# ZooMEISTER/vickers-hardness-Unet

Hardware: AMD Instinct MI355X
Metric: 512x512 images/sec (train fwd+bwd) (higher is better)
Workload: dtype bf16

## Files before the change

### include/vk_unet.h

```cpp
#ifndef VK_UNET_H
#define VK_UNET_H

#include <stddef.h>
#include <stdint.h>

#ifdef __cplusplus
extern "C" {
#endif

#define VK_ABI_VERSION 1
#define VK_STATS_REPLICAS 32

typedef enum { VK_F32 = 0, VK_BF16 = 1, VK_F16 = 2 } vk_dtype;

enum { VK_OK = 0, VK_ERR_ARG = -1, VK_ERR_STATE = -2, VK_ERR_UNSUPPORTED = -3 };

int vk_version(void);
const char* vk_last_error_string(void);
int vk_has_gfx950_code(void);
int vk_probe_mfma_rate(int iters, int waves_per_simd, float* sink, double* flops_out, void* stream);
int vk_set_reserved_cus(int n);
int vk_debug_hold_cus(int workgroups, int threads, int lds_bytes, int microseconds, const void* traffic, size_t traffic_bytes,
                      float* sink, void* stream);

// ... 27 lines not shown
int vk_conv_dgrad_pool2(const vk_conv_desc* d, const void* w, void* y_half, void* y1, int split_k1, int accumulate,
                        void* stream);

int vk_halo_pack(vk_dtype dtype, int rows, int red, const void* src, void* dst, void* stream);
int vk_conv_uses_halo_pack(const vk_conv_desc* d);
int vk_conv_fwd_packed(const vk_conv_desc* d, const void* w_halo, void* y, void* y1, int split_k1, int accumulate, double* stats,
                       void* stream);

#define VK_SPLITK_WORKSPACE_BYTES (32u << 20)
int vk_conv_fwd_splitk(const vk_conv_desc* d, const void* w_halo, void* y, void* workspace, size_t workspace_bytes, void* stream);

typedef struct {
  const void* z;
  const float* scale;
  const float* shift;
  double* sums;
  const void* mask;
  int accumulate;
} vk_bnr;

int vk_conv_dgrad_fused(const vk_conv_desc* d, const void* w, void* y, void* y1, int split_k1, int pool2, const vk_bnr* bnr,
                        void* stream);

int vk_conv1x1_fwd(const vk_conv_desc* d, const void* w, void* y, int accumulate, double* stats, void* stream);
int vk_conv1x1_wgrad(const vk_conv_desc* d, const void* dz, float* dw, void* workspace, size_t workspace_bytes, void* stream);

int vk_stem_fwd(vk_dtype dtype, int N, int H, int W, const void* x4, const void* wp, void* y, double* stats,
                void* stream);

#define VK_WGRAD_WORKSPACE_BYTES (64u << 20)
int vk_conv_wgrad(const vk_conv_desc* d, const void* dz, float* dw, void* workspace, size_t workspace_bytes, void* stream);
#define VK_WGRAD_BATCH_TABLE_BYTES (128u << 10)
int vk_conv_wgrad_batch_supports(const vk_conv_desc* d);
int vk_conv_wgrad_batch(const vk_conv_desc* descs, const void* const* dz, float* const* dw, int n, int workgroups, void* tables,
                        size_t tables_bytes, void* workspace, size_t workspace_bytes, void* stream);
int vk_stem_wgrad(vk_dtype dtype, int N, int H, int W, const void* x4, const void* dz, float* dw_krsc3, void* workspace,
                  size_t workspace_bytes, void* stream);
int vk_stem_wgrad_bn(vk_dtype dtype, int N, int H, int W, const void* x4, const void* g, const void* z, const float* coef_abc,
                     float* dw_krsc3, void* workspace, size_t workspace_bytes, void* stream);
int vk_stem_wgrad_c(vk_dtype dtype, int N, int H, int W, int cin, const void* x4, const void* dz, float* dw_krsc, void* workspace,
                    size_t workspace_bytes, void* stream);
int vk_stem_wgrad_bn_c(vk_dtype dtype, int N, int H, int W, int cin, const void* x4, const void* g, const void* z, const float* coef_abc,
                       float* dw_krsc, void* workspace, size_t workspace_bytes, void* stream);
int vk_conv_bwd_onepass(const vk_conv_desc* d_fwd, const void* g, const void* z, const float* coef_abc, const void* w_dgrad, void* y,
                        const vk_bnr* bnr, float* dw, void* workspace, size_t workspace_bytes, void* stream);
int vk_stem_dgrad(vk_dtype dtype, int N, int H, int W, const void* g, const void* z, const float* coef_abc, const float* w_krsc3,
                  float* dx, void* stream);
int vk_stem_dgrad_c(vk_dtype dtype, int N, int H, int W, int cin, const void* g, const void* z, const float* coef_abc, const float* w_krsc,
// ... 587 lines not shown
  int dims[4];
  int ndim;
  int64_t offset;
  int64_t numel;
} vk_tensor_info;

int vk_unet_create(const vk_unet_config* cfg, vk_unet** out);
int vk_unet_create_ex(const vk_unet_config* cfg, int classes, vk_unet** out);
int vk_unet_num_classes(const vk_unet* h);
#define VK_ENC_RESNET18 18
#define VK_ENC_RESNET34 34
#define VK_ENC_RESNET50 50
int vk_unet_create_enc(const vk_unet_config* cfg, int classes, int encoder, vk_unet** out);
int vk_unet_encoder(const vk_unet* h);
int vk_unet_create_in(const vk_unet_config* cfg, int classes, int encoder, int in_channels, vk_unet** out);
int vk_unet_in_channels(const vk_unet* h);
void vk_unet_destroy(vk_unet* h);
int vk_unet_set_side_stream(vk_unet* h, int enable);
int vk_unet_num_tensors(const vk_unet* h);
int vk_unet_tensor_info(const vk_unet* h, int index, vk_tensor_info* out);
int64_t vk_unet_param_numel(const vk_unet* h);
int64_t vk_unet_buffer_numel(const vk_unet* h);
int64_t vk_unet_workspace_bytes(const vk_unet* h);
int vk_unet_num_buckets(const vk_unet* h);
int vk_unet_bucket_range(const vk_unet* h, int bucket, int64_t* elem_begin, int64_t* elem_end);

int vk_unet_bind(vk_unet* h, float* params, float* grads, float* bn_buffers, int64_t* nbt, void* workspace,
                 size_t workspace_bytes);
int vk_unet_refresh_weights(vk_unet* h, void* stream);

int vk_unet_forward(vk_unet* h, const float* x, float* logits, int training, void* stream);
int vk_unet_loss(vk_unet* h, const float* logits, const float* target, float* loss_out, float grad_scale,
                 float w_bce, float w_dice, void* stream);
#define VK_LOSS_BINARY 0
#define VK_LOSS_MULTILABEL 1
#define VK_LOSS_MULTICLASS 2
int vk_unet_loss_ex(vk_unet* h, int mode, const void* logits, const void* target, float* loss_out, float grad_scale, float w_ce,
                    float w_dice, void* stream);
int vk_unet_loss_cfg(vk_unet* h, const vk_seg_loss_cfg* cfg, const void* logits, const void* target, float* loss_out,
                     float grad_scale, void* stream);
int vk_unet_loss_lovasz(vk_unet* h, const vk_seg_loss_cfg* seg_cfg, const vk_lovasz_cfg* lovasz_cfg, float w_lovasz, const void* logits,
                        const void* target, void* workspace, size_t workspace_bytes, float* loss_out, float grad_scale, void* stream);
int vk_unet_loss_kp(vk_unet* h, const vk_seg_loss_cfg* seg_cfg, const vk_kp_loss_cfg* kp_cfg, const void* logits, const void* target,
                    void* workspace, size_t workspace_bytes, float* loss_out, float grad_scale, void* stream);
int vk_unet_backward(vk_unet* h, const float* dlogits, int stage_begin, int stage_end, void* stream);
int vk_unet_set_trainable(vk_unet* h, const uint8_t* flags, int n);
// ... 20 lines not shown
```

### vickers-hardness-unet_amd/_lib.py

```python
from __future__ import annotations

import ctypes as C
import os
import subprocess
from pathlib import Path

PKG_DIR = Path(__file__).resolve().parent
LIB_PATH = Path(os.environ["VK_LIB"]) if os.environ.get("VK_LIB") else PKG_DIR / "libvkunet.so"
CSRC = PKG_DIR / "csrc"

VK_F32, VK_BF16, VK_F16 = 0, 1, 2
VK_LOSS_BINARY, VK_LOSS_MULTILABEL, VK_LOSS_MULTICLASS = 0, 1, 2
VK_ENC_RESNET18, VK_ENC_RESNET34, VK_ENC_RESNET50 = 18, 34, 50
VK_ADAMW_MAX_GROUPS = 8
VK_NORM_L2, VK_NORM_INF = 0, 1
VK_TILE_MAX_ORIGINS, VK_TILE_MAX_SIDE = 64, 4096
VK_BLEND_PROB, VK_BLEND_LOGIT = 0, 1
VK_PATCH_FORCE_GENERAL = 1


class VkError(RuntimeError):
    pass


# ... 264 lines not shown
vp, ci, cf, cd, sz, i64 = C.c_void_p, C.c_int, C.c_float, C.c_double, C.c_size_t, C.c_int64
P = C.POINTER

SIGNATURES = {
    "vk_version": (ci, []),
    "vk_last_error_string": (C.c_char_p, []),
    "vk_has_gfx950_code": (ci, []),
    "vk_probe_mfma_rate": (ci, [ci, ci, vp, P(C.c_double), vp]),
    "vk_set_reserved_cus": (ci, [ci]),
    "vk_debug_hold_cus": (ci, [ci, ci, ci, ci, vp, sz, vp, vp]),
    "vk_debug_set_stamp_buffer": (ci, [vp]),
    "vk_prof_enable": (ci, [ci]),
    "vk_prof_collect": (ci, [C.c_char_p, sz]),
    "vk_conv_fwd": (ci, [P(vk_conv_desc), vp, vp, vp, ci, ci, vp, vp]),
    "vk_conv_dgrad_pool2": (ci, [P(vk_conv_desc), vp, vp, vp, ci, ci, vp]),
    "vk_conv_dgrad_fused": (ci, [P(vk_conv_desc), vp, vp, vp, ci, ci, P(vk_bnr), vp]),
    "vk_head_bwd_fused": (ci, [ci, ci, ci, ci, P(vk_src), vp, vp, vp, vp, vp, P(vk_bnr), vp, sz, vp]),
    "vk_halo_pack": (ci, [ci, ci, ci, vp, vp, vp]),
    "vk_conv_uses_halo_pack": (ci, [P(vk_conv_desc)]),
    "vk_conv_fwd_packed": (ci, [P(vk_conv_desc), vp, vp, vp, ci, ci, vp, vp]),
    "vk_conv_fwd_splitk": (ci, [P(vk_conv_desc), vp, vp, vp, sz, vp]),
    "vk_stem_fwd": (ci, [ci, ci, ci, ci, vp, vp, vp, vp, vp]),
    "vk_conv_wgrad": (ci, [P(vk_conv_desc), vp, vp, vp, sz, vp]),
    "vk_conv1x1_fwd": (ci, [P(vk_conv_desc), vp, vp, ci, vp, vp]),
    "vk_conv1x1_wgrad": (ci, [P(vk_conv_desc), vp, vp, vp, sz, vp]),
    "vk_conv_wgrad_batch_supports": (ci, [P(vk_conv_desc)]),
    "vk_conv_wgrad_batch": (ci, [P(vk_conv_desc), P(vp), P(vp), ci, ci, vp, sz, vp, sz, vp]),
    "vk_stem_wgrad": (ci, [ci, ci, ci, ci, vp, vp, vp, vp, sz, vp]),
    "vk_stem_wgrad_bn": (ci, [ci, ci, ci, ci, vp, vp, vp, vp, vp, vp, sz, vp]),
    "vk_stem_wgrad_c": (ci, [ci, ci, ci, ci, ci, vp, vp, vp, vp, sz, vp]),
    "vk_stem_wgrad_bn_c": (ci, [ci, ci, ci, ci, ci, vp, vp, vp, vp, vp, vp, sz, vp]),
    "vk_conv_bwd_onepass": (ci, [P(vk_conv_desc), vp, vp, vp, vp, vp, P(vk_bnr), vp, vp, sz, vp]),
    "vk_stem_dgrad": (ci, [ci, ci, ci, ci, vp, vp, vp, vp, vp, vp]),
    "vk_stem_dgrad_c": (ci, [ci, ci, ci, ci, ci, vp, vp, vp, vp, vp, vp]),
    "vk_letterbox_preprocess": (ci, [P(vk_letterbox_desc), vp, vp, vp]),
    "vk_letterbox_postprocess_mask": (ci, [P(vk_letterbox_desc), vp, cf, vp, vp]),
    "vk_letterbox_postprocess_prob": (ci, [P(vk_letterbox_desc), vp, vp, vp]),
    "vk_letterbox_postprocess_labels": (ci, [P(vk_letterbox_desc), ci, vp, vp, vp]),
    "vk_letterbox_postprocess_mask_multi": (ci, [P(vk_letterbox_desc), ci, vp, cf, vp, vp]),
    "vk_letterbox_postprocess_prob_multi": (ci, [P(vk_letterbox_desc), ci, ci, vp, vp, vp]),
    "vk_tile_preprocess": (ci, [P(vk_tile_desc), vp, vp, vp]),
    "vk_tile_blend": (ci, [P(vk_tile_desc), ci, vp, cf, vp, vp, vp]),
    "vk_geom_workspace_bytes": (i64, [P(vk_geom_desc), ci]),
    "vk_geom_minarearect": (ci, [P(vk_geom_desc), ci, vp, vp, vp, vp, vp, sz, vp]),
    "vk_geom_quadrilateral": (ci, [P(vk_geom_desc), ci, ci, vp, vp, vp, vp, vp, sz, vp]),
    "vk_geom_slot_map": (ci, [P(vk_geom_desc), ci, vp, sz, vp, vp]),
    "vk_letterbox_u8": (ci, [P(vk_letterbox_desc), vp, vp, vp]),
    "vk_letterbox_mask_u8": (ci, [P(vk_letterbox_desc), vp, vp, vp]),
# ... 76 lines not shown
    "vk_adamw_step_amp": (ci, [sz, vp, vp, vp, vp, cf, cf, cf, cf, cf, vp, cf, vp, vp, vp, vp, ci, vp]),
    "vk_adamw_segment_blocks": (ci, [ci, P(i64), P(C.c_int32), ci]),
    "vk_adamw_step_amp_segments": (ci, [ci, vp, ci, vp, vp, vp, vp, vp, cf, cf, cf, cf, cf, vp, cf, vp, vp, vp, vp]),
    "vk_adamw_step_groups": (ci, [ci, vp, vp, ci, vp, vp, vp, vp, vp, ci, P(vk_adamw_group), vp, cf, vp, vp, vp, vp, vp]),
    "vk_grad_norm_segments": (ci, [ci, vp, ci, vp, vp, ci, cf, cf, vp, vp, vp]),
    "vk_avg_update": (ci, [ci, P(vk_avg_range), vk_avg_rule, vp, vp, vp, vp]),
    "vk_avg_swap": (ci, [ci, P(vk_avg_range), vp]),
    "vk_adamw_step_amp_avg": (ci, [sz, vp, vp, vp, vp, cf, cf, cf, cf, cf, vp, cf, vp, vp, vp, vp, ci, vp, vp, vk_avg_rule, vp, vp, vp, sz,
                                   vp]),
    "vk_unet_create": (ci, [P(vk_unet_config), P(vp)]),
    "vk_unet_create_ex": (ci, [P(vk_unet_config), ci, P(vp)]),
    "vk_unet_num_classes": (ci, [vp]),
    "vk_unet_create_enc": (ci, [P(vk_unet_config), ci, ci, P(vp)]),
    "vk_unet_encoder": (ci, [vp]),
    "vk_unet_create_in": (ci, [P(vk_unet_config), ci, ci, ci, P(vp)]),
    "vk_unet_in_channels": (ci, [vp]),
    "vk_unet_destroy": (None, [vp]),
    "vk_unet_set_side_stream": (ci, [vp, ci]),
    "vk_unet_num_tensors": (ci, [vp]),
    "vk_unet_tensor_info": (ci, [vp, ci, P(vk_tensor_info)]),
    "vk_unet_param_numel": (i64, [vp]),
    "vk_unet_buffer_numel": (i64, [vp]),
    "vk_unet_workspace_bytes": (i64, [vp]),
    "vk_unet_num_buckets": (ci, [vp]),
    "vk_unet_bucket_range": (ci, [vp, ci, P(i64), P(i64)]),
    "vk_unet_bind": (ci, [vp, vp, vp, vp, vp, vp, sz]),
    "vk_unet_refresh_weights": (ci, [vp, vp]),
    "vk_unet_forward": (ci, [vp, vp, vp, ci, vp]),
    "vk_unet_loss": (ci, [vp, vp, vp, vp, cf, cf, cf, vp]),
    "vk_unet_loss_ex": (ci, [vp, ci, vp, vp, vp, cf, cf, cf, vp]),
    "vk_unet_loss_cfg": (ci, [vp, P(vk_seg_loss_cfg), vp, vp, vp, cf, vp]),
    "vk_unet_loss_lovasz": (ci, [vp, P(vk_seg_loss_cfg), P(vk_lovasz_cfg), cf, vp, vp, vp, sz, vp, cf, vp]),
    "vk_unet_loss_kp": (ci, [vp, P(vk_seg_loss_cfg), P(vk_kp_loss_cfg), vp, vp, vp, sz, vp, cf, vp]),
    "vk_unet_backward": (ci, [vp, vp, ci, ci, vp]),
    "vk_unet_set_trainable": (ci, [vp, P(C.c_uint8), ci]),
    "vk_unet_set_bn_frozen": (ci, [vp, P(C.c_uint8), ci]),
    "vk_unet_set_input_grad": (ci, [vp, vp]),
    "vk_unet_zero_grad": (ci, [vp, vp]),
    "vk_unet_debug_tensor": (ci, [vp, C.c_char_p, P(vp), P(ci * 4)]),
    "vk_comm_unique_id": (ci, [vp]),
    "vk_comm_init": (ci, [ci, ci, vp, P(vp)]),
    "vk_comm_world": (ci, [vp]),
    "vk_allreduce_bucket": (ci, [vp, vp, sz, vp]),
    "vk_comm_broadcast": (ci, [vp, vp, sz, ci, vp]),
    "vk_comm_destroy": (ci, [vp]),
}
# ... 73 lines not shown
```

### vickers-hardness-unet_amd/csrc/elementwise.hip

```cpp
#include <math.h>

#include "vk_common.h"

namespace vk {

constexpr int kWideC = 2048;
static inline int channel_grid(int blocks, int cv) {
  int g = cv, r = 256;
  while (r) { const int t = g % r; g = r; r = t; }
  const int m = cv / g;
  return (blocks + m - 1) / m * m;
}

template <typename T>
__global__ void k_input_transform(int N, int cin, int H, int W, const float* __restrict__ x, T* __restrict__ x4) {
  const size_t HW = (size_t)H * W;
  const float* xn = x + (size_t)blockIdx.y * cin * HW;
  T* on = x4 + (size_t)blockIdx.y * HW * 4;
  for (size_t hw = blockIdx.x * (size_t)blockDim.x + threadIdx.x; hw < HW; hw += (size_t)gridDim.x * blockDim.x) {
    const float r = xn[hw], g = cin > 1 ? xn[HW + hw] : 0.f, b = cin > 2 ? xn[2 * HW + hw] : 0.f, a = cin > 3 ? xn[3 * HW + hw] : 0.f;
    if constexpr (sizeof(T) == 4) {
      *reinterpret_cast<f32x4_t*>(on + hw * 4) = f32x4_t{r, g, b, a};
    } else {
      float f[8] = {r, g, b, a, 0.f, 0.f, 0.f, 0.f};
// ... 438 lines not shown
                                                              const float* __restrict__ save_mean, const float* __restrict__ save_invstd,
                                                              float* dgamma, float* dbeta, float* coef) {
  const int c = blockIdx.x * 8 + (threadIdx.x >> 5);
  const int q = threadIdx.x & 31;
  double sg = 0.0, sgz = 0.0;
  if (c < C) {
    sg = sums[(size_t)q * 2 * C + c];
    sgz = sums[(size_t)q * 2 * C + C + c];
  }
#pragma unroll
  for (int o = 16; o > 0; o >>= 1) {
    sg += __shfl_xor(sg, o, 64);
    sgz += __shfl_xor(sgz, o, 64);
  }
  if (q != 0 || c >= C) return;
  const float r = save_invstd[c];
  dgamma[c] += (float)((double)r * (sgz - (double)save_mean[c] * sg));
  dbeta[c] += (float)sg;
  coef[c] = gamma[c] * r;
  coef[C + c] = 0.f;
  coef[2 * C + c] = 0.f;
}

template <typename T, int MASK, int MAXC>
__global__ __launch_bounds__(256) void k_bn_bwd_apply(size_t pixels, int C, const T* __restrict__ dy, const T* __restrict__ z,
                                                      const float* __restrict__ scale, const float* __restrict__ shift, const T* __restrict__ mask_src,
                                                      const float* __restrict__ coef, const double* __restrict__ sums, double count,
                                                      const float* __restrict__ gamma, const float* __restrict__ save_mean,
                                                      const float* __restrict__ save_invstd, float* dgamma, float* dbeta, T* __restrict__ dz, T* g_out,
                                                      int g_acc) {
  constexpr int VE = ElemTraits<T>::kVec;
  constexpr int U = 2;
  const int CV = C / VE;
  const size_t total = pixels * CV;
  const size_t stride = (size_t)gridDim.x * blockDim.x;
  const size_t t0 = blockIdx.x * (size_t)blockDim.x + threadIdx.x;
  const int c0 = (int)(t0 % CV) * VE;
  __shared__ float cf[3][MAXC];
  if (coef) {
    for (int c = threadIdx.x; c < C; c += blockDim.x) {
      cf[0][c] = coef[c];
      cf[1][c] = coef[C + c];
      cf[2][c] = coef[2 * C + c];
    }
  } else {
    static_assert(VK_STATS_REPLICAS == 32, "replica mapping");
    for (int c8 = threadIdx.x; c8 < C * 8; c8 += blockDim.x) {
      const int c = c8 >> 3, q0 = (c8 & 7) * 4;
      double sg = 0.0, sgz = 0.0;
#pragma unroll
      for (int q = 0; q < 4; ++q) {
        sg += sums[(size_t)(q0 + q) * 2 * C + c];
        sgz += sums[(size_t)(q0 + q) * 2 * C + C + c];
      }
#pragma unroll
      for (int o = 4; o > 0; o >>= 1) {
        sg += __shfl_xor(sg, o, 64);
        sgz += __shfl_xor(sgz, o, 64);
      }
      if ((c8 & 7) == 0) {
        const float mu = save_mean[c], r = save_invstd[c], ga = gamma[c];
        const float d = (float)(sgz - (double)mu * sg);
        const float sgf = (float)sg, inv = (float)(1.0 / count);
        const float dg = r * d;
        const float a = ga * r, b = -a * r * dg * inv;
        cf[0][c] = a;
        cf[1][c] = b;
        cf[2][c] = -a * sgf * inv - b * mu;
        if (blockIdx.x == 0) {
          dgamma[c] += dg;
          dbeta[c] += sgf;
        }
      }
    }
  }
  __syncthreads();
  float sc[VE], sh[VE], ca[VE], cb[VE], cc[VE];
#pragma unroll
  for (int j = 0; j < VE; ++j) {
    sc[j] = (MASK == 1) ? scale[c0 + j] : 1.f;
    sh[j] = (MASK == 1) ? shift[c0 + j] : 0.f;
    ca[j] = cf[0][c0 + j];
    cb[j] = cf[1][c0 + j];
    cc[j] = cf[2][c0 + j];
  }
  for (size_t i = t0; i < total; i += U * stride) {
    float g[U][VE], zf[U][VE];
#pragma unroll
    for (int u = 0; u < U; ++u)
      if (i + u * stride < total) masked_grad<T, MASK>(dy, z, mask_src, (i + u * stride) * VE, sc, sh, g[u], zf[u]);
#pragma unroll
    for (int u = 0; u < U; ++u) {
      const size_t k = i + u * stride;
      if (k >= total) continue;
      float o[VE];
#pragma unroll
      for (int j = 0; j < VE; ++j) o[j] = fmaf(ca[j], g[u][j], fmaf(cb[j], zf[u][j], cc[j]));
      *reinterpret_cast<u32x4_t*>(dz + k * VE) = Vec16<T>::pack(o);
      if (g_out) {
        u32x4_t* gp = reinterpret_cast<u32x4_t*>(g_out + k * VE);
        if (g_acc) {
          float old[VE];
          Vec16<T>::unpack(*gp, old);
#pragma unroll
          for (int j = 0; j < VE; ++j) g[u][j] += old[j];
        }
        *gp = Vec16<T>::pack(g[u]);
      }
    }
  }
}

template <typename T>
__global__ void k_upsample2x_bwd(int N, int H, int W, int C, const T* __restrict__ d_up, T* __restrict__ d_low, int acc) {
  constexpr int VE = ElemTraits<T>::kVec;
  const int Hl = H / 2, Wl = W / 2, CV = C / VE;
  const size_t total = (size_t)N * Hl * Wl * CV;
  for (size_t i = blockIdx.x * (size_t)blockDim.x + threadIdx.x; i < total; i += (size_t)gridDim.x * blockDim.x) {
    const int cv = (int)(i % CV);
    size_t t = i / CV;
    const int wl = (int)(t % Wl);
    t /= Wl;
    const int hl = (int)(t % Hl);
    const int n = (int)(t / Hl);
    float s[VE];
#pragma unroll
    for (int j = 0; j < VE; ++j) s[j] = 0.f;
#pragma unroll
    for (int a = 0; a < 2; ++a)
#pragma unroll
      for (int b = 0; b < 2; ++b) {
// ... 744 lines not shown
}

extern "C" int vk_bn_bwd_coeffs_frozen(int C, const double* sums, const float* gamma, const float* running_mean, const float* running_invstd,
                                       float* dgamma, float* dbeta, float* coef_abc, void* stream) {
  VK_CHECK_ARG(sums && gamma && running_mean && running_invstd && dgamma && dbeta && coef_abc, "vk_bn_bwd_coeffs_frozen: null argument");
  vkh::ProfScope ps_("bn_bwd_coeffs_frozen", (hipStream_t)stream, 0.0, (double)C * 48.0);
  hipLaunchKernelGGL(k_bn_bwd_coeffs_frozen, dim3((C + 7) / 8), dim3(256), 0, (hipStream_t)stream, C, sums, gamma, running_mean,
                     running_invstd, dgamma, dbeta, coef_abc);
  VK_CHECK_HIP(hipGetLastError());
  return VK_OK;
}

struct BnApplyArgs {
  size_t pixels; int C; const void* dy; const void* z; int mask_mode; const float* scale; const float* shift; const void* mask_src;
  const float* coef; const double* sums; double count; const float* gamma; const float* mean; const float* invstd; float* dgamma; float* dbeta;
  void* dz; void* g_out; int g_acc;
};

template <typename T>
static int launch_bn_bwd_apply(const BnApplyArgs& a, hipStream_t st) {
  const int CV = a.C / ElemTraits<T>::kVec;
  const bool wide = a.C > 512;
  dim3 grid(channel_grid(grid_for(a.pixels * CV / 2 + 1), CV)), block(256);
  if (wide) {
#define VK_APPLY_W(M) hipLaunchKernelGGL((k_bn_bwd_apply<T, M, kWideC>), grid, block, 0, st, a.pixels, a.C, (const T*)a.dy, (const T*)a.z, a.scale, \
    a.shift, (const T*)a.mask_src, a.coef, a.sums, a.count, a.gamma, a.mean, a.invstd, a.dgamma, a.dbeta, (T*)a.dz, (T*)a.g_out, a.g_acc)
    if (a.mask_mode == 0) VK_APPLY_W(0);
    else if (a.mask_mode == 1) VK_APPLY_W(1);
    else VK_APPLY_W(2);
#undef VK_APPLY_W
    return VK_OK;
  }
#define VK_APPLY(M) hipLaunchKernelGGL((k_bn_bwd_apply<T, M, 512>), grid, block, 0, st, a.pixels, a.C, (const T*)a.dy, (const T*)a.z, a.scale, a.shift, \
    (const T*)a.mask_src, a.coef, a.sums, a.count, a.gamma, a.mean, a.invstd, a.dgamma, a.dbeta, (T*)a.dz, (T*)a.g_out, a.g_acc)
  if (a.mask_mode == 0) VK_APPLY(0);
  else if (a.mask_mode == 1) VK_APPLY(1);
  else VK_APPLY(2);
#undef VK_APPLY
  return VK_OK;
}

static int bn_bwd_apply_common(vk_dtype dtype, const BnApplyArgs& a, void* stream) {
  VK_CHECK_ARG(a.dy && a.z && a.dz && (a.coef || (a.sums && a.gamma && a.mean && a.invstd && a.dgamma && a.dbeta)), "vk_bn_bwd_apply: null argument");
  VK_CHECK_ARG(a.mask_mode >= 0 && a.mask_mode <= 2, "vk_bn_bwd_apply: mask_mode %d", a.mask_mode);
  VK_CHECK_ARG(a.mask_mode != 1 || (a.scale && a.shift), "vk_bn_bwd_apply: mask_mode 1 needs scale/shift");
  VK_CHECK_ARG(a.mask_mode != 2 || a.mask_src, "vk_bn_bwd_apply: mask_mode 2 needs mask_src");
  if (const int rc = check_flat_channels("vk_bn_bwd_apply", a.C)) return rc;
  hipStream_t st = (hipStream_t)stream;
  vkh::ProfScope ps_("bn_bwd_apply", st, 0.0, (double)a.pixels * a.C * (dtype == VK_F32 ? 4.0 : 2.0) * ((a.mask_mode == 2 ? 4.0 : 3.0) + (a.g_out ? (a.g_acc ? 2.0 : 1.0) : 0.0)));
  DISPATCH_T(dtype, launch_bn_bwd_apply<T>(a, st));
  VK_CHECK_HIP(hipGetLastError());
  return VK_OK;
}

extern "C" int vk_bn_bwd_apply(vk_dtype dtype, size_t pixels, int C, const void* dy, const void* z, int mask_mode,
                               const float* scale, const float* shift, const void* mask_src, const float* coef_abc, void* dz,
                               void* g_out, int g_accumulate, void* stream) {
  VK_CHECK_ARG(coef_abc, "vk_bn_bwd_apply: null coefficients");
  BnApplyArgs a{pixels, C, dy, z, mask_mode, scale, shift, mask_src, coef_abc, nullptr, 1.0, nullptr, nullptr, nullptr, nullptr, nullptr, dz, g_out, g_accumulate};
  return bn_bwd_apply_common(dtype, a, stream);
}

extern "C" int vk_bn_bwd_apply_fused(vk_dtype dtype, size_t pixels, int C, const void* dy, const void* z, int mask_mode,
                                     const float* scale, const float* shift, const void* mask_src, const double* sums, double count,
                                     const float* gamma, const float* save_mean, const float* save_invstd, float* dgamma, float* dbeta,
                                     void* dz, void* g_out, int g_accumulate, void* stream) {
  BnApplyArgs a{pixels, C, dy, z, mask_mode, scale, shift, mask_src, nullptr, sums, count, gamma, save_mean, save_invstd, dgamma, dbeta, dz, g_out, g_accumulate};
  return bn_bwd_apply_common(dtype, a, stream);
}

// ... 105 lines not shown
```

### vickers-hardness-unet_amd/csrc/engine.hip

```cpp
#include <stdarg.h>
#include <stdio.h>
#include <stdlib.h>
#include <string.h>

#include <algorithm>
#include <atomic>
#include <map>
#include <mutex>
#include <string>
#include <vector>

#include "conv_host.h"

namespace vkh {
static thread_local char g_err[512] = "";
void set_error(const char* fmt, ...) {
  va_list ap;
  va_start(ap, fmt);
  vsnprintf(g_err, sizeof(g_err), fmt, ap);
  va_end(ap);
}

struct ProfRec {
  std::string tag;
// ... 380 lines not shown
  std::vector<vk_tensor_info> infos;
  int n_ptensors = 0;
  std::vector<uint8_t> trainable;
  int last_rank = 0;
  uint64_t bn_frozen = 0, bn_frozen_fwd = 0;
  float* dx_in = nullptr;
  int input_rank = 0;
  unsigned mask_version = 0;
  std::vector<ConvL> convs;
  std::vector<BnL> bns;
  std::vector<BlockL> blocks;
  std::vector<DecL> decs;
  int stem_conv = -1, head_conv = -1;
  int layer_last_block[4];
  int64_t n_params = 0, n_bufs = 0, n_dgrad = 0;
  int64_t head_w_off = 0, head_b_off = 0;
  std::vector<std::pair<int64_t, int64_t>> buckets;
  size_t ws_bytes = 0;
  size_t off_x4 = 0, off_pool = 0, off_argmax = 0, off_gpool = 0, off_dup = 0, off_dlogits = 0, off_loss_sums = 0;
  size_t off_stats = 0, off_bsums = 0, stats_bytes = 0, off_farena = 0, farena_floats = 0, off_wf = 0, off_wd = 0, off_wstem = 0;
  size_t off_tab_pack = 0, off_tab_bn = 0, off_wslab = 0, off_wh = 0, off_tab_halo = 0, off_splitk = 0, splitk_bytes = 0;
  std::vector<HaloPackEntry> halo_tab;
  std::vector<size_t> off_z, off_g, off_out, off_gout;
  std::vector<char> g_prereduced;
  std::vector<char> tail_prereduced;
  float* params = nullptr;
  float* grads = nullptr;
  float* bufs = nullptr;
  int64_t* nbt = nullptr;
  char* ws = nullptr;
  bool bound = false;
  hipStream_t side = nullptr;
  hipEvent_t ev_fork = nullptr, ev_join = nullptr;
  bool side_dirty = false;
  struct WItem {
    vk_conv_desc d;
    const void* dz;
    float* dw;
  };
  struct WPlan {
    bool built = false;
    int target = 0, n = 0;
    unsigned version = 0;
    vk::WgradBatchPlan plan;
  };
  std::vector<WItem> pending;
// ... 201 lines not shown
  }
  bn(h->stem_conv); conv(h->stem_conv);
  h->input_rank = r;
  h->trainable.assign((size_t)h->n_ptensors, 1);
  h->last_rank = r - 1;
}

void update_last_rank(vk_unet* h) {
  h->last_rank = -1;
  for (const ConvL& c : h->convs) {
    if (trains(h, c.w_t) || (c.b_t >= 0 && trains(h, c.b_t))) h->last_rank = std::max(h->last_rank, c.rank);
  }
  for (const BnL& b : h->bns) {
    if (trains(h, b.g_t) || trains(h, b.b_t)) h->last_rank = std::max(h->last_rank, b.rank);
  }
  if (h->dx_in) h->last_rank = h->input_rank;
}

size_t grad_scratch_floats(const vk_unet* h) {
  if (h->enc->code != VK_ENC_RESNET34) return align_up(2 * (size_t)h->sink_c + 145 * (size_t)h->classes, 64);
  return h->classes == 1 ? kGradScratchFloats : align_up(1024 + 145 * (size_t)h->classes, 64);
}

void layout_workspace(vk_unet* h) {
  const int N = h->cfg.N, S = h->cfg.size, SW = h->cfg.width, eb = h->eb;
  const bool tr = h->cfg.training != 0;
  size_t off = 0;
  auto take = [&](size_t bytes) {
    const size_t o = off;
    off = align_up(off + bytes, 256);
    return o;
  };
  h->off_x4 = take((size_t)N * S * SW * 4 * eb);
  h->g_prereduced.assign(h->convs.size(), 0);
  h->tail_prereduced.assign(h->blocks.size(), 0);
  h->off_z.resize(h->convs.size());
  h->off_g.assign(h->convs.size(), 0);
  for (size_t i = 0; i < h->convs.size(); ++i) {
    const ConvL& c = h->convs[i];
    if ((int)i == h->head_conv) { h->off_z[i] = 0; continue; }
    const size_t bytes = (size_t)N * c.Hout * c.Wout * c.K * eb;
    h->off_z[i] = take(bytes);
    if (tr) h->off_g[i] = take(bytes);
  }
  h->off_pool = take((size_t)N * (S / 4) * (SW / 4) * 64 * eb);
  h->off_argmax = take((size_t)N * (S / 4) * (SW / 4) * 64);
  if (tr) h->off_gpool = take((size_t)N * (S / 4) * (SW / 4) * 64 * eb);
  h->off_out.resize(h->blocks.size());
  h->off_gout.assign(h->blocks.size(), 0);
  for (size_t b = 0; b < h->blocks.size(); ++b) {
    const BlockL& k = h->blocks[b];
    const size_t bytes = (size_t)N * k.Hout * k.Wout * k.C * eb;
    h->off_out[b] = take(bytes);
    if (tr) h->off_gout[b] = take(bytes);
  }
  if (tr) {
    size_t mx = 0;
    for (const DecL& d : h->decs) mx = std::max(mx, (size_t)N * d.H * d.W * d.Cup * eb);
    h->off_dup = take(mx);
    h->off_dlogits = take((size_t)N * h->classes * S * SW * 4);
  }
  h->off_loss_sums = take(8 * sizeof(double));
  size_t st = 0, fl = 0;
  for (BnL& b : h->bns) {
    st += 2 * (size_t)b.C * sizeof(double) * VK_STATS_REPLICAS;
    b.arena_off = (int64_t)fl;
    fl += 7 * (size_t)b.C;
  }
  h->stats_bytes = st;
  h->off_stats = take(st);
  h->off_bsums = take(st);
  h->farena_floats = fl;
  h->off_farena = take(fl * sizeof(float));
  h->off_wf = (eb == 4) ? 0 : take((size_t)h->n_params * eb);
  h->off_wd = tr ? take((size_t)h->n_dgrad * eb) : 0;
  h->off_wh = take((size_t)h->n_params * eb);
  h->off_tab_halo = take(2 * h->convs.size() * sizeof(HaloPackEntry));
  h->off_wstem = take(64 * 7 * 32 * eb);
// ... 10 lines not shown
    h->off_mloss = take(h->mloss_bytes);
  }
  h->sloss_bytes = vk_seg_loss_workspace_bytes(N, h->classes, S * SW);
  h->off_sloss = take(h->sloss_bytes);
  h->ws_bytes = off;
}

void assign_pointers(vk_unet* h) {
  char* ws = h->ws;
  h->debug.clear();
  const int N = h->cfg.N;
  for (size_t i = 0; i < h->convs.size(); ++i) {
    ConvL& c = h->convs[i];
    if ((int)i == h->head_conv) continue;
    c.z = ws + h->off_z[i];
    c.g = h->cfg.training ? ws + h->off_g[i] : nullptr;
    h->debug["z:" + c.name] = {c.z, {N, c.Hout, c.Wout, c.K}};
    if (c.g) h->debug["g:" + c.name] = {c.g, {N, c.Hout, c.Wout, c.K}};
  }
  for (size_t b = 0; b < h->blocks.size(); ++b) {
    BlockL& k = h->blocks[b];
    k.out = ws + h->off_out[b];
    k.gout = h->cfg.training ? ws + h->off_gout[b] : nullptr;
    const std::string nm = h->convs[k.conv1].name.substr(0, h->convs[k.conv1].name.size() - 6);
    h->debug["out:" + nm] = {k.out, {N, k.Hout, k.Wout, k.C}};
    if (k.gout) h->debug["gout:" + nm] = {k.gout, {N, k.Hout, k.Wout, k.C}};
  }
  const int S = h->cfg.size, SW = h->cfg.width;
  h->debug["x4"] = {ws + h->off_x4, {N, S, SW, 4}};
  h->debug["pool"] = {ws + h->off_pool, {N, S / 4, SW / 4, 64}};
  if (h->cfg.training) {
    h->debug["gpool"] = {ws + h->off_gpool, {N, S / 4, SW / 4, 64}};
    if (h->classes == 1) h->debug["dlogits"] = {ws + h->off_dlogits, {N, S, SW, 1}};
    else h->debug["dlogits"] = {ws + h->off_dlogits, {N, h->classes, S, SW}};
  }
  double* sp = (double*)(ws + h->off_stats);
  double* bp = (double*)(ws + h->off_bsums);
  float* fa = (float*)(ws + h->off_farena);
  for (BnL& b : h->bns) {
    b.stats = sp;
    b.bsums = bp;
    sp += 2 * b.C * VK_STATS_REPLICAS;
    bp += 2 * b.C * VK_STATS_REPLICAS;
    float* f = fa + b.arena_off;
    b.scale = f;
    b.shift = f + b.C;
    b.mean = f + 2 * b.C;
// ... 149 lines not shown
extern "C" int vk_unet_num_classes(const vk_unet* h) { return h ? h->classes : 0; }
extern "C" int vk_unet_encoder(const vk_unet* h) { return h ? h->enc->code : 0; }
extern "C" int vk_unet_in_channels(const vk_unet* h) { return h ? h->in_channels : 0; }

extern "C" void vk_unet_destroy(vk_unet* h) {
  if (!h) return;
  if (h->side) {
    (void)hipStreamSynchronize(h->side);
    (void)hipEventDestroy(h->ev_fork);
    (void)hipEventDestroy(h->ev_join);
    (void)hipStreamDestroy(h->side);
  }
  delete h;
}
extern "C" int vk_unet_num_tensors(const vk_unet* h) { return h ? (int)h->infos.size() : 0; }
extern "C" int vk_unet_tensor_info(const vk_unet* h, int index, vk_tensor_info* out) {
  VK_CHECK_ARG(h && out && index >= 0 && index < (int)h->infos.size(), "vk_unet_tensor_info: bad index %d", index);
  *out = h->infos[index];
  return VK_OK;
}
extern "C" int64_t vk_unet_param_numel(const vk_unet* h) { return h ? h->n_params : 0; }
extern "C" int64_t vk_unet_buffer_numel(const vk_unet* h) { return h ? h->n_bufs : 0; }
extern "C" int64_t vk_unet_workspace_bytes(const vk_unet* h) { return h ? (int64_t)h->ws_bytes : 0; }
extern "C" int vk_unet_num_buckets(const vk_unet* h) { return h ? (int)h->buckets.size() : 0; }
extern "C" int vk_unet_bucket_range(const vk_unet* h, int bucket, int64_t* b, int64_t* e) {
  VK_CHECK_ARG(h && b && e && bucket >= 0 && bucket < (int)h->buckets.size(), "vk_unet_bucket_range: bad bucket %d", bucket);
  *b = h->buckets[bucket].first;
  *e = h->buckets[bucket].second;
  return VK_OK;
}

extern "C" int vk_unet_bind(vk_unet* h, float* params, float* grads, float* bn_buffers, int64_t* nbt, void* workspace,
                            size_t workspace_bytes) {
  VK_CHECK_ARG(h && params && bn_buffers && nbt && workspace, "vk_unet_bind: null argument");
  VK_CHECK_ARG(!h->cfg.training || grads, "vk_unet_bind: a training plan needs a gradient buffer");
  VK_CHECK_ARG(workspace_bytes >= h->ws_bytes, "vk_unet_bind: workspace too small (%zu < %zu)", workspace_bytes, h->ws_bytes);
  VK_CHECK_ARG(((uintptr_t)workspace & 255) == 0 && ((uintptr_t)params & 15) == 0, "vk_unet_bind: buffers must be 256-byte (workspace) / 16-byte (params) aligned");
  h->params = params; h->grads = grads; h->bufs = bn_buffers; h->nbt = nbt; h->ws = (char*)workspace;
  for (auto& st_ : h->wplans) { st_[0].built = false; st_[1].built = false; }
  h->pending.clear();
  assign_pointers(h);
  h->halo_tab.clear();
  {
    auto plain = [&](int C) { vk_src s = null_src(); s.ptr = h->ws; s.C = C; return s; };
    auto fwd_uses = [&](ConvL& c, int C0, int C1, int up) {
      vk_src s0 = plain(C0), s1 = C1 ? plain(C1) : null_src();
// ... 494 lines not shown
std::pair<Act, void*> block_input(vk_unet* h, int bi) {
  if (bi == 0) return {Act{h->ws + h->off_pool, 64, nullptr, nullptr, 0}, h->ws + h->off_gpool};
  BlockL& pb = h->blocks[bi - 1];
  return {Act{pb.out, pb.C, nullptr, nullptr, 0}, pb.gout};
}

int backward_block(vk_unet* h, int bi, hipStream_t st) {
  BlockL& k = h->blocks[bi];
  ConvL& c1 = h->convs[k.conv1];
  ConvL& c2 = h->convs[k.conv2];
  BnL& b2 = h->bns[c2.bn];
  const vk_dtype dt = h->cfg.dtype;
  const size_t pixels = (size_t)h->cfg.N * k.Hout * k.Wout;
  if (!need_from(h, b2.rank)) {
    h->tail_prereduced[(size_t)bi] = 0;
    return VK_OK;
  }
  const auto [xin, gin] = block_input(h, bi);
  const bool pre = h->tail_prereduced[(size_t)bi] != 0;
  h->tail_prereduced[(size_t)bi] = 0;
  if (bi > 0) h->tail_prereduced[(size_t)bi - 1] = 0;
  const int mm = pre ? 0 : 2;
  if (!pre && bn_sums_needed(h, b2)) RET_IF(vk_bn_bwd_reduce(dt, pixels, k.C, k.gout, c2.z, 2, nullptr, nullptr, k.out, b2.bsums, st));
  if (k.convd < 0) {
    RET_IF(bn_bwd_phase2(h, b2, k.C, pixels, k.gout, c2.z, mm, k.out, c2.g, gin, k.in_has_grad_first ? 1 : 0, st));
  } else {
    ConvL& cd = h->convs[k.convd];
    BnL& bd = h->bns[cd.bn];
    RET_IF(bn_bwd_phase2(h, b2, k.C, pixels, k.gout, c2.z, mm, k.out, c2.g, nullptr, 0, st));
    if (bn_sums_needed(h, bd)) RET_IF(vk_bn_bwd_reduce(dt, pixels, k.C, k.gout, cd.z, mm, nullptr, nullptr, k.out, bd.bsums, st));
    RET_IF(bn_bwd_phase2(h, bd, k.C, pixels, k.gout, cd.z, mm, k.out, cd.g, nullptr, 0, st));
  }
  const bool into1 = need_from(h, h->bns[c1.bn].rank);
  bool fused1 = false;
  if (into1) RET_IF(conv_dgrad_into(h, c2, c1, &fused1, st));
  if (trains(h, c2.w_t)) RET_IF(conv_wgrad(h, c2, to_src(bn_act(h, c1)), null_src(), st));
  if (!into1) return k.convd >= 0 && trains(h, h->convs[k.convd].w_t) ? conv_wgrad(h, h->convs[k.convd], to_src(xin), null_src(), st) : VK_OK;
  RET_IF(bn_relu_bwd_inplace(h, c1, fused1, st));
  const bool into_gin = need_from(h, c1.rank + 1);
  bool tail_fused = false;
  const int tail_maxc = getenv("VK_TAIL_BNR_MAXC") ? atoi(getenv("VK_TAIL_BNR_MAXC")) : 1 << 20;
  if (into_gin && k.convd < 0 && bi > 0 && c1.halo_dg && k.C <= tail_maxc && !getenv("VK_NO_TAIL_BNR_FUSION")) {
    BlockL& pb = h->blocks[bi - 1];
    ConvL& pc2 = h->convs[pb.conv2];
    vk_conv_desc dd = dgrad_desc(h, c1);
    vk_bnr r;
    r.z = pc2.z; r.scale = nullptr; r.shift = nullptr; r.sums = h->bns[pc2.bn].bsums; r.mask = pb.out; r.accumulate = 1;
// ... 195 lines not shown
```

Before: 3094.

## Alias residual gradient buffers across same-shape blocks and apply BN backward in place

Lets consecutive residual blocks of the same stage share one gradient-output buffer, and lets the pool gradient reuse the first block's buffer. A new in-place BN backward apply kernel writes the masked gradient back into the shared buffer, so the block-input gradient needs no separate buffer and no accumulate pass. This shrinks the workspace and cuts memory traffic (no extra accumulate read/write), at the cost of tighter aliasing rules that could corrupt gradients if an ordering assumption breaks. It also adds a workspace-offset query API.

```diff
diff --git a/include/vk_unet.h b/include/vk_unet.h
--- a/include/vk_unet.h
+++ b/include/vk_unet.h
@@ -73,8 +73,7 @@
 int vk_conv_dgrad_fused(const vk_conv_desc* d, const void* w, void* y, void* y1, int split_k1, int pool2, const vk_bnr* bnr,
                         void* stream);
 
-int vk_conv1x1_fwd(const vk_conv_desc* d, const void* w, void* y, int accumulate, double* stats, void* stream);
-int vk_conv1x1_wgrad(const vk_conv_desc* d, const void* dz, float* dw, void* workspace, size_t workspace_bytes, void* stream);
+int vk_conv1x1_fwd(const vk_conv_desc* d, const void* w, void* y, int accumulate, double* stats, void* stream);int vk_conv1x1_wgrad(const vk_conv_desc* d, const void* dz, float* dw, void* workspace, size_t workspace_bytes, void* stream);
 
 int vk_stem_fwd(vk_dtype dtype, int N, int H, int W, const void* x4, const void* wp, void* y, double* stats,
                 void* stream);
@@ -708,6 +707,7 @@
 int64_t vk_unet_param_numel(const vk_unet* h);
 int64_t vk_unet_buffer_numel(const vk_unet* h);
 int64_t vk_unet_workspace_bytes(const vk_unet* h);
+int vk_unet_workspace_offset(const vk_unet* h, const char* name, int64_t* offset);
 int vk_unet_num_buckets(const vk_unet* h);
 int vk_unet_bucket_range(const vk_unet* h, int bucket, int64_t* elem_begin, int64_t* elem_end);
 
diff --git a/vickers-hardness-unet_amd/_lib.py b/vickers-hardness-unet_amd/_lib.py
--- a/vickers-hardness-unet_amd/_lib.py
+++ b/vickers-hardness-unet_amd/_lib.py
@@ -310,8 +310,7 @@
     "vk_conv_fwd_splitk": (ci, [P(vk_conv_desc), vp, vp, vp, sz, vp]),
     "vk_stem_fwd": (ci, [ci, ci, ci, ci, vp, vp, vp, vp, vp]),
     "vk_conv_wgrad": (ci, [P(vk_conv_desc), vp, vp, vp, sz, vp]),
-    "vk_conv1x1_fwd": (ci, [P(vk_conv_desc), vp, vp, ci, vp, vp]),
-    "vk_conv1x1_wgrad": (ci, [P(vk_conv_desc), vp, vp, vp, sz, vp]),
+    "vk_conv1x1_fwd": (ci, [P(vk_conv_desc), vp, vp, ci, vp, vp]),    "vk_conv1x1_wgrad": (ci, [P(vk_conv_desc), vp, vp, vp, sz, vp]),
     "vk_conv_wgrad_batch_supports": (ci, [P(vk_conv_desc)]),
     "vk_conv_wgrad_batch": (ci, [P(vk_conv_desc), P(vp), P(vp), ci, ci, vp, sz, vp, sz, vp]),
     "vk_stem_wgrad": (ci, [ci, ci, ci, ci, vp, vp, vp, vp, sz, vp]),
@@ -434,6 +433,7 @@
     "vk_unet_param_numel": (i64, [vp]),
     "vk_unet_buffer_numel": (i64, [vp]),
     "vk_unet_workspace_bytes": (i64, [vp]),
+    "vk_unet_workspace_offset": (ci, [vp, C.c_char_p, P(i64)]),
     "vk_unet_num_buckets": (ci, [vp]),
     "vk_unet_bucket_range": (ci, [vp, ci, P(i64), P(i64)]),
     "vk_unet_bind": (ci, [vp, vp, vp, vp, vp, vp, sz]),
diff --git a/vickers-hardness-unet_amd/csrc/elementwise.hip b/vickers-hardness-unet_amd/csrc/elementwise.hip
--- a/vickers-hardness-unet_amd/csrc/elementwise.hip
+++ b/vickers-hardness-unet_amd/csrc/elementwise.hip
@@ -484,6 +484,49 @@
   coef[2 * C + c] = 0.f;
 }
 
+template <int MAXC>
+__device__ __forceinline__ void bn_apply_coef_table(float (&cf)[3][MAXC], int C, const float* __restrict__ coef, const double* __restrict__ sums,
+                                                    double count, const float* __restrict__ gamma, const float* __restrict__ save_mean,
+                                                    const float* __restrict__ save_invstd, float* dgamma, float* dbeta) {
+  if (coef) {
+    for (int c = threadIdx.x; c < C; c += blockDim.x) {
+      cf[0][c] = coef[c];
+      cf[1][c] = coef[C + c];
+      cf[2][c] = coef[2 * C + c];
+    }
+  } else {
+    static_assert(VK_STATS_REPLICAS == 32, "replica mapping");
+    for (int c8 = threadIdx.x; c8 < C * 8; c8 += blockDim.x) {
+      const int c = c8 >> 3, q0 = (c8 & 7) * 4;
+      double sg = 0.0, sgz = 0.0;
+#pragma unroll
+      for (int q = 0; q < 4; ++q) {
+        sg += sums[(size_t)(q0 + q) * 2 * C + c];
+        sgz += sums[(size_t)(q0 + q) * 2 * C + C + c];
+      }
+#pragma unroll
+      for (int o = 4; o > 0; o >>= 1) {
+        sg += __shfl_xor(sg, o, 64);
+        sgz += __shfl_xor(sgz, o, 64);
+      }
+      if ((c8 & 7) == 0) {
+        const float mu = save_mean[c], r = save_invstd[c], ga = gamma[c];
+        const float d = (float)(sgz - (double)mu * sg);
+        const float sgf = (float)sg, inv = (float)(1.0 / count);
+        const float dg = r * d;
+        const float a = ga * r, b = -a * r * dg * inv;
+        cf[0][c] = a;
+        cf[1][c] = b;
+        cf[2][c] = -a * sgf * inv - b * mu;
+        if (blockIdx.x == 0) {
+          dgamma[c] += dg;
+          dbeta[c] += sgf;
+        }
+      }
+    }
+  }
+}
+
 template <typename T, int MASK, int MAXC>
 __global__ __launch_bounds__(256) void k_bn_bwd_apply(size_t pixels, int C, const T* __restrict__ dy, const T* __restrict__ z,
                                                       const float* __restrict__ scale, const float* __restrict__ shift, const T* __restrict__ mask_src,
@@ -499,43 +542,7 @@
   const size_t t0 = blockIdx.x * (size_t)blockDim.x + threadIdx.x;
   const int c0 = (int)(t0 % CV) * VE;
   __shared__ float cf[3][MAXC];
-  if (coef) {
-    for (int c = threadIdx.x; c < C; c += blockDim.x) {
-      cf[0][c] = coef[c];
-      cf[1][c] = coef[C + c];
-      cf[2][c] = coef[2 * C + c];
-    }
-  } else {
-    static_assert(VK_STATS_REPLICAS == 32, "replica mapping");
-    for (int c8 = threadIdx.x; c8 < C * 8; c8 += blockDim.x) {
-      const int c = c8 >> 3, q0 = (c8 & 7) * 4;
-      double sg = 0.0, sgz = 0.0;
-#pragma unroll
-      for (int q = 0; q < 4; ++q) {
-        sg += sums[(size_t)(q0 + q) * 2 * C + c];
-        sgz += sums[(size_t)(q0 + q) * 2 * C + C + c];
-      }
-#pragma unroll
-      for (int o = 4; o > 0; o >>= 1) {
-        sg += __shfl_xor(sg, o, 64);
-        sgz += __shfl_xor(sgz, o, 64);
-      }
-      if ((c8 & 7) == 0) {
-        const float mu = save_mean[c], r = save_invstd[c], ga = gamma[c];
-        const float d = (float)(sgz - (double)mu * sg);
-        const float sgf = (float)sg, inv = (float)(1.0 / count);
-        const float dg = r * d;
-        const float a = ga * r, b = -a * r * dg * inv;
-        cf[0][c] = a;
-        cf[1][c] = b;
-        cf[2][c] = -a * sgf * inv - b * mu;
-        if (blockIdx.x == 0) {
-          dgamma[c] += dg;
-          dbeta[c] += sgf;
-        }
-      }
-    }
-  }
+  bn_apply_coef_table<MAXC>(cf, C, coef, sums, count, gamma, save_mean, save_invstd, dgamma, dbeta);
   __syncthreads();
   float sc[VE], sh[VE], ca[VE], cb[VE], cc[VE];
 #pragma unroll
@@ -569,6 +576,46 @@
         }
         *gp = Vec16<T>::pack(g[u]);
       }
+    }
+  }
+}
+
+template <typename T, int MAXC>
+__global__ __launch_bounds__(256) void k_bn_bwd_apply_inplace(size_t pixels, int C, T* g_io, const T* __restrict__ z, const T* __restrict__ mask_src,
+                                                              const float* __restrict__ coef, const double* __restrict__ sums, double count,
+                                                              const float* __restrict__ gamma, const float* __restrict__ save_mean,
+                                                              const float* __restrict__ save_invstd, float* dgamma, float* dbeta, T* __restrict__ dz) {
+  constexpr int VE = ElemTraits<T>::kVec;
+  constexpr int U = 2;
+  const int CV = C / VE;
+  const size_t total = pixels * CV;
+  const size_t stride = (size_t)gridDim.x * blockDim.x;
+  const size_t t0 = blockIdx.x * (size_t)blockDim.x + threadIdx.x;
+  const int c0 = (int)(t0 % CV) * VE;
+  __shared__ float cf[3][MAXC];
+  bn_apply_coef_table<MAXC>(cf, C, coef, sums, count, gamma, save_mean, save_invstd, dgamma, dbeta);
+  __syncthreads();
+  float ca[VE], cb[VE], cc[VE];
+#pragma unroll
+  for (int j = 0; j < VE; ++j) {
+    ca[j] = cf[0][c0 + j];
+    cb[j] = cf[1][c0 + j];
+    cc[j] = cf[2][c0 + j];
+  }
+  for (size_t i = t0; i < total; i += U * stride) {
+    float g[U][VE], zf[U][VE];
+#pragma unroll
+    for (int u = 0; u < U; ++u)
+      if (i + u * stride < total) masked_grad<T, 2>(g_io, z, mask_src, (i + u * stride) * VE, nullptr, nullptr, g[u], zf[u]);
+#pragma unroll
+    for (int u = 0; u < U; ++u) {
+      const size_t k = i + u * stride;
+      if (k >= total) continue;
+      float o[VE];
+#pragma unroll
+      for (int j = 0; j < VE; ++j) o[j] = fmaf(ca[j], g[u][j], fmaf(cb[j], zf[u][j], cc[j]));
+      *reinterpret_cast<u32x4_t*>(dz + k * VE) = Vec16<T>::pack(o);
+      *reinterpret_cast<u32x4_t*>(g_io + k * VE) = Vec16<T>::pack(g[u]);
     }
   }
 }
@@ -1359,6 +1406,14 @@
   const int CV = a.C / ElemTraits<T>::kVec;
   const bool wide = a.C > 512;
   dim3 grid(channel_grid(grid_for(a.pixels * CV / 2 + 1), CV)), block(256);
+  if (a.g_out == a.dy) {
+#define VK_APPLY_I(MAXC) hipLaunchKernelGGL((k_bn_bwd_apply_inplace<T, MAXC>), grid, block, 0, st, a.pixels, a.C, (T*)a.g_out, (const T*)a.z, \
+    (const T*)a.mask_src, a.coef, a.sums, a.count, a.gamma, a.mean, a.invstd, a.dgamma, a.dbeta, (T*)a.dz)
+    if (wide) VK_APPLY_I(kWideC);
+    else VK_APPLY_I(512);
+#undef VK_APPLY_I
+    return VK_OK;
+  }
   if (wide) {
 #define VK_APPLY_W(M) hipLaunchKernelGGL((k_bn_bwd_apply<T, M, kWideC>), grid, block, 0, st, a.pixels, a.C, (const T*)a.dy, (const T*)a.z, a.scale, \
     a.shift, (const T*)a.mask_src, a.coef, a.sums, a.count, a.gamma, a.mean, a.invstd, a.dgamma, a.dbeta, (T*)a.dz, (T*)a.g_out, a.g_acc)
@@ -1383,6 +1438,8 @@
   VK_CHECK_ARG(a.mask_mode != 1 || (a.scale && a.shift), "vk_bn_bwd_apply: mask_mode 1 needs scale/shift");
   VK_CHECK_ARG(a.mask_mode != 2 || a.mask_src, "vk_bn_bwd_apply: mask_mode 2 needs mask_src");
   if (const int rc = check_flat_channels("vk_bn_bwd_apply", a.C)) return rc;
+  VK_CHECK_ARG(a.g_out != a.dy || (a.mask_mode == 2 && !a.g_acc), "vk_bn_bwd_apply: g_out == dy (in place) needs mask_mode 2 and no accumulate");
+  VK_CHECK_ARG(a.dz != a.dy || a.g_out != a.dy, "vk_bn_bwd_apply: dz and g_out both in place");
   hipStream_t st = (hipStream_t)stream;
   vkh::ProfScope ps_("bn_bwd_apply", st, 0.0, (double)a.pixels * a.C * (dtype == VK_F32 ? 4.0 : 2.0) * ((a.mask_mode == 2 ? 4.0 : 3.0) + (a.g_out ? (a.g_acc ? 2.0 : 1.0) : 0.0)));
   DISPATCH_T(dtype, launch_bn_bwd_apply<T>(a, st));
diff --git a/vickers-hardness-unet_amd/csrc/engine.hip b/vickers-hardness-unet_amd/csrc/engine.hip
--- a/vickers-hardness-unet_amd/csrc/engine.hip
+++ b/vickers-hardness-unet_amd/csrc/engine.hip
@@ -426,6 +426,7 @@
   size_t off_tab_pack = 0, off_tab_bn = 0, off_wslab = 0, off_wh = 0, off_tab_halo = 0, off_splitk = 0, splitk_bytes = 0;
   std::vector<HaloPackEntry> halo_tab;
   std::vector<size_t> off_z, off_g, off_out, off_gout;
+  bool gout_alias = false;
   std::vector<char> g_prereduced;
   std::vector<char> tail_prereduced;
   float* params = nullptr;
@@ -673,6 +674,11 @@
   return h->classes == 1 ? kGradScratchFloats : align_up(1024 + 145 * (size_t)h->classes, 64);
 }
 
+std::string block_name(const vk_unet* h, const BlockL& k) {
+  const std::string& c = h->convs[(size_t)k.conv1].name;
+  return c.substr(0, c.size() - 6);
+}
+
 void layout_workspace(vk_unet* h) {
   const int N = h->cfg.N, S = h->cfg.size, SW = h->cfg.width, eb = h->eb;
   const bool tr = h->cfg.training != 0;
@@ -696,15 +702,22 @@
   }
   h->off_pool = take((size_t)N * (S / 4) * (SW / 4) * 64 * eb);
   h->off_argmax = take((size_t)N * (S / 4) * (SW / 4) * 64);
-  if (tr) h->off_gpool = take((size_t)N * (S / 4) * (SW / 4) * 64 * eb);
+  h->gout_alias = tr && !h->enc->bottleneck && !getenv("VK_NO_GOUT_ALIAS");
+  const bool gpool_alias = h->gout_alias && !h->blocks.empty() && h->blocks[0].convd < 0 && h->blocks[0].C == 64 &&
+                           h->blocks[0].Hout == S / 4 && h->blocks[0].Wout == SW / 4;
+  if (tr && !gpool_alias) h->off_gpool = take((size_t)N * (S / 4) * (SW / 4) * 64 * eb);
   h->off_out.resize(h->blocks.size());
   h->off_gout.assign(h->blocks.size(), 0);
   for (size_t b = 0; b < h->blocks.size(); ++b) {
     const BlockL& k = h->blocks[b];
     const size_t bytes = (size_t)N * k.Hout * k.Wout * k.C * eb;
     h->off_out[b] = take(bytes);
-    if (tr) h->off_gout[b] = take(bytes);
-  }
+    if (!tr) continue;
+    const bool same_stage = h->gout_alias && b > 0 && k.convd < 0 && h->blocks[b - 1].C == k.C && h->blocks[b - 1].Hout == k.Hout &&
+                            h->blocks[b - 1].Wout == k.Wout;
+    h->off_gout[b] = same_stage ? h->off_gout[b - 1] : take(bytes);
+  }
+  if (gpool_alias) h->off_gpool = h->off_gout[0];
   if (tr) {
     size_t mx = 0;
     for (const DecL& d : h->decs) mx = std::max(mx, (size_t)N * d.H * d.W * d.Cup * eb);
@@ -761,7 +774,7 @@
     BlockL& k = h->blocks[b];
     k.out = ws + h->off_out[b];
     k.gout = h->cfg.training ? ws + h->off_gout[b] : nullptr;
-    const std::string nm = h->convs[k.conv1].name.substr(0, h->convs[k.conv1].name.size() - 6);
+    const std::string nm = block_name(h, k);
     h->debug["out:" + nm] = {k.out, {N, k.Hout, k.Wout, k.C}};
     if (k.gout) h->debug["gout:" + nm] = {k.gout, {N, k.Hout, k.Wout, k.C}};
   }
@@ -957,6 +970,18 @@
 extern "C" int64_t vk_unet_param_numel(const vk_unet* h) { return h ? h->n_params : 0; }
 extern "C" int64_t vk_unet_buffer_numel(const vk_unet* h) { return h ? h->n_bufs : 0; }
 extern "C" int64_t vk_unet_workspace_bytes(const vk_unet* h) { return h ? (int64_t)h->ws_bytes : 0; }
+extern "C" int vk_unet_workspace_offset(const vk_unet* h, const char* name, int64_t* offset) {
+  VK_CHECK_ARG(h && name && offset, "vk_unet_workspace_offset: null argument");
+  const std::string s(name);
+  if (s == "gpool" && h->cfg.training) { *offset = (int64_t)h->off_gpool; return VK_OK; }
+  for (size_t b = 0; b < h->blocks.size(); ++b) {
+    const std::string nm = block_name(h, h->blocks[b]);
+    if (s == "out:" + nm) { *offset = (int64_t)h->off_out[b]; return VK_OK; }
+    if (s == "gout:" + nm && h->cfg.training) { *offset = (int64_t)h->off_gout[b]; return VK_OK; }
+  }
+  vkh::set_error("vk_unet_workspace_offset: unknown tensor '%s'", name);
+  return VK_ERR_ARG;
+}
 extern "C" int vk_unet_num_buckets(const vk_unet* h) { return h ? (int)h->buckets.size() : 0; }
 extern "C" int vk_unet_bucket_range(const vk_unet* h, int bucket, int64_t* b, int64_t* e) {
   VK_CHECK_ARG(h && b && e && bucket >= 0 && bucket < (int)h->buckets.size(), "vk_unet_bucket_range: bad bucket %d", bucket);
@@ -1497,7 +1522,9 @@
   if (bi > 0) h->tail_prereduced[(size_t)bi - 1] = 0;
   const int mm = pre ? 0 : 2;
   if (!pre && bn_sums_needed(h, b2)) RET_IF(vk_bn_bwd_reduce(dt, pixels, k.C, k.gout, c2.z, 2, nullptr, nullptr, k.out, b2.bsums, st));
-  if (k.convd < 0) {
+  if (k.convd < 0 && gin == k.gout) {
+    RET_IF(bn_bwd_phase2(h, b2, k.C, pixels, k.gout, c2.z, mm, k.out, c2.g, pre ? nullptr : k.gout, 0, st));
+  } else if (k.convd < 0) {
     RET_IF(bn_bwd_phase2(h, b2, k.C, pixels, k.gout, c2.z, mm, k.out, c2.g, gin, k.in_has_grad_first ? 1 : 0, st));
   } else {
     ConvL& cd = h->convs[k.convd];
```

Result: no change. 3115 (median of 6 runs) (+0.7%).
